# dusk-network/dusk-zerocaf

Measured on AMD Instinct MI355X. Metric: 252-bit Edwards variable-base scalar-muls/sec (batched, strict bit-exact mode), higher is better.
Workload: dtype u64 (nine 29-bit limbs in u32 registers, 64-bit multiply-accumulate columns); 1 GPU; 2^20 EdwardsPoint variable-base scalar-mul, random 252-bit scalars (BASELINE configs[2]); mode=strict (reference formula sequence, identical X:Y:Z:T limbs)

## Files before the change

### dusk_zerocaf_amd/csrc/zc_curve.hip.h

```cpp
#pragma once
#include "zc_arith.hip.h"

namespace zc {

typedef ModP FP;

struct pt {
    fe X, Y, Z, T;
};

template <int N>
struct exp_program {
    u32 e[N];
};
template <int N>
constexpr exp_program<N> make_program(const u32 (&src)[N])
{
    exp_program<N> p{};
    for (int i = 0; i < N; i++) p.e[i] = src[i];
    return p;
}
__device__ __constant__ exp_program<ModP::PROG_INV_LEN> ZC_PROG_INV = make_program(ModP::PROG_INV);
__device__ __constant__ exp_program<ModP::PROG_P58_LEN> ZC_PROG_P58 = make_program(ModP::PROG_P58);

// ... 587 lines not shown
    r.Ym = fp_sub(p.Y, p.X);
    r.Yp = fe_add(p.Y, p.X);
    r.Z = p.Z;
    r.T = p.T;
    return r;
}
ZC_DI ptm ptm_select(bool c, const ptm& a, const ptm& b)
{
    ptm r;
    r.Ym = fe_select(c, a.Ym, b.Ym);
    r.Yp = fe_select(c, a.Yp, b.Yp);
    r.Z = fe_select(c, a.Z, b.Z);
    r.T = fe_select(c, a.T, b.T);
    return r;
}
template <bool ILP = false>
ZC_DI ptm ptm_add(const ptm& p, const ptm& q)
{
    auto fp_mul = [](const fe& x, const fe& y) { return ILP ? mont_mul_ilp<FP>(x, y) : mont_mul<FP>(x, y); };
    const fe M = fp_mul(p.Ym, q.Ym);
    const fe P = fp_mul(p.Yp, q.Yp);
    const fe C = fp_mul(fp_mul_d(p.T), q.T);
    const fe D = fp_mul(p.Z, q.Z);
    const fe E = fe_sub_half<FP>(P, M);
    const fe H = fe_sub_lazy<FP>(P, E);
    const fe F = fe_sub_lazy<FP>(D, C);
    const fe G = fe_add(D, C);
    const fe X3 = fp_mul(E, F), Y3 = fp_mul(G, H);
    ptm r;
    r.Ym = fp_sub(Y3, X3);
    r.Yp = fe_add(Y3, X3);
    r.Z = fp_mul(F, G);
    r.T = fp_mul(E, H);
    return r;
}
ZC_DI pt ptm_to_pt(const ptm& p)
{
    const fe half = fe_const<FP>(ModP::INV2_M);
    pt r;
    r.X = fp_mul(fp_sub(p.Yp, fe_reduce<FP>(p.Ym)), half);
    r.Y = fp_mul(fe_add(p.Yp, p.Ym), half);
    r.Z = p.Z;
    r.T = p.T;
    return r;
}
ZC_DI pt pt_neg(const pt& p)
{
    pt r;
    r.X = fe_reduce<FP>(fp_neg(p.X));
    r.Y = p.Y;
    r.Z = p.Z;
    r.T = fe_reduce<FP>(fp_neg(p.T));
    return r;
}
ZC_DI pt pt_load(const u64* __restrict__ p)
{
    pt r;
    r.X = fe_load_mont<FP>(p);
    r.Y = fe_load_mont<FP>(p + 5);
    r.Z = fe_load_mont<FP>(p + 10);
    r.T = fe_load_mont<FP>(p + 15);
    return r;
}
ZC_DI void pt_store(u64* __restrict__ o, const pt& p)
{
    fe_store_canon<FP>(o, p.X);
    fe_store_canon<FP>(o + 5, p.Y);
    fe_store_canon<FP>(o + 10, p.Z);
    fe_store_canon<FP>(o + 15, p.T);
}

ZC_DI void scalar_effective(u64 (&l)[5])
{
#pragma unroll
    for (int j = 0; j < 5; j++) l[j] &= M52;
    const u64 low48 = ((u64)1 << 48) - 1;
    const u32 hi = (u32)(l[4] >> 48);
    if (hi) {
        const int tz = __builtin_ctz(hi);
        const bool stops_early = (l[1] | l[2] | l[3] | (l[4] & low48)) == 0 && l[0] < ((u64)1 << tz);
        if (stops_early) l[4] &= low48;
    }
}
ZC_DI void load_scalar(u64 (&l)[5], const u64* __restrict__ p)
{
    load5(l, p);
    scalar_effective(l);
}

ZC_DI void scalar_to_words(u32* __restrict__ sk, int stride, const u64 (&l)[5], int& nbits)
{
    u32 w[9];
#pragma unroll
    for (int k = 0; k < 9; k++) {
        const int bit = 32 * k, idx = bit / 52, sh = bit % 52;
        u64 x = (idx < 5) ? ((l[idx] & M52) >> sh) : 0;
        if (sh + 32 > 52 && idx + 1 < 5) x |= (l[idx + 1] & M52) << (52 - sh);
        w[k] = (u32)x;
    }
    w[8] &= 0xFu;
    nbits = 0;
#pragma unroll
    for (int k = 0; k < 9; k++) {
        if (w[k]) nbits = 32 * k + (32 - __builtin_clz(w[k]));
        sk[k * stride] = w[k];
    }
}

template <bool ILP = false>
ZC_DI pt scalar_mul_unified(const pt& P, const u32* __restrict__ sk, int stride, int nbits)
{
    ptm N = ptm_from_pt(P), Q = ptm_from_pt(pt_identity());
    int pos = 0;
    u32 cur = sk[0];
    bool pend = (cur & 1) != 0;
    bool active = nbits > 0;
    while (active) {
        const ptm lhs = ptm_select(pend, Q, N);
        const ptm r = ptm_add<ILP>(lhs, N);
        if (pend) {
            Q = r;
            pend = false;
            active = pos < nbits - 1;
        } else {
            N = r;
            pos++;
            if ((pos & 31) == 0) cur = sk[(pos >> 5) * stride];
            pend = ((cur >> (pos & 31)) & 1) != 0;
        }
    }
    return ptm_to_pt(Q);
}

ZC_DI ptm ptm_double_valid(const ptm& n)
{
    const fe M = mont_sqr<FP>(n.Ym);
    const fe P = mont_sqr<FP>(n.Yp);
    const fe D = mont_sqr<FP>(n.Z);
    const fe G = mont_mul<FP>(n.Ym, n.Yp);
    const fe E = fe_sub_half<FP>(P, M);
    const fe H = fe_sub_lazy<FP>(P, E);
    const fe F = fp_sub(fe_add(D, D), G);
    const fe X3 = mont_mul<FP>(E, F), Y3 = mont_mul<FP>(G, H);
    ptm r;
    r.Ym = fp_sub(Y3, X3);
    r.Yp = fe_add(Y3, X3);
    r.Z = mont_mul<FP>(F, G);
    r.T = mont_mul<FP>(E, H);
    return r;
}
ZC_DI bool pt_doubling_identities_hold(const pt& p, const ptm& n)
{
    const fe lhs = mont_mul<FP>(n.Ym, n.Yp);
    const fe rhs = fe_add(mont_sqr<FP>(p.Z), mont_mul<FP>(fe_const<FP>(ModP::D_M), mont_sqr<FP>(p.T)));
    return fp_eq(rhs, lhs) && fp_eq(mont_mul<FP>(p.T, p.Z), mont_mul<FP>(p.X, p.Y));
}
struct sm_lane {
    int pos, nbits;
    u32 cur;
    bool taken;
    bool has_stash;
    bool active;
};
ZC_DI sm_lane sm_lane_init(const u32* __restrict__ sk, int nbits)
{
    sm_lane L;
    L.pos = 0;
    L.nbits = nbits;
    L.cur = sk[0];
    L.taken = false;
    L.has_stash = false;
    L.active = nbits > 0;
    return L;
}
ZC_DI bool sm_bit_pending(const sm_lane& L) { return ((L.cur >> (L.pos & 31)) & 1) != 0 && !L.taken; }
ZC_DI bool sm_at_top(const sm_lane& L) { return L.active && L.pos >= L.nbits - 1; }
ZC_DI bool sm_tile_wants_d_step(bool any_active, bool any_at_top) { return any_active && !any_at_top; }
ZC_DI void sm_lane_advance(sm_lane& L, const u32* __restrict__ sk, int stride)
{
    L.pos++;
    if ((L.pos & 31) == 0) L.cur = sk[(L.pos >> 5) * stride];
    L.taken = false;
}
ZC_DI void sm_g_commit(ptm& dst, const u32 (&d)[9], const fe& Y3, const fe& X3, const fe& Z3, const fe& T3)
{
    u32 mask = M29, zero = 0;
    ZC_OPAQUE(mask);
    ZC_OPAQUE(zero);
#pragma unroll
    for (int i = 0; i < 9; i++) {
        dst.Ym.v[i] = i < 8 ? d[i] & mask : d[i];
        dst.Yp.v[i] = Y3.v[i] + X3.v[i] + zero;
    }
    dst.Z = Z3;
    dst.T = T3;
}
template <class STASH>
ZC_DI void sm_g_step(sm_lane& L, ptm& N, ptm& Q, const STASH& S, const u32* __restrict__ sk, int stride)
{
    const bool from_stash = L.active && L.has_stash;
    const bool add = L.active && (L.has_stash || sm_bit_pending(L));
    const bool dbl = L.active && !add;
    u32 d[9];
    fe X3, Y3, Z3, T3;
    {
        const ptm lhs = ptm_select(add, Q, N);
        const fe M = mont_mul<FP>(lhs.Ym, fe_select(from_stash, S.get(0), N.Ym));
        const fe P = mont_mul<FP>(lhs.Yp, fe_select(from_stash, S.get(1), N.Yp));
        const fe C = mont_mul<FP>(fp_mul_d(lhs.T), fe_select(from_stash, S.get(3), N.T));
        const fe D = mont_mul<FP>(lhs.Z, fe_select(from_stash, S.get(2), N.Z));
        const fe E = fe_sub_half<FP>(P, M);
        const fe H = fe_sub_lazy<FP>(P, E);
        const fe F = fe_sub_lazy<FP>(D, C);
        const fe G = fe_add(D, C);
        X3 = mont_mul<FP>(E, F);
        Y3 = mont_mul<FP>(G, H);
        Z3 = mont_mul<FP>(F, G);
        T3 = mont_mul<FP>(E, H);
    }
    for (int i = 0; i < 9; i++) ZC_ASSERT(X3.v[i] <= FP::BIAS[i] && Y3.v[i] < (1u << 31));
#pragma unroll
    for (int i = 0; i < 9; i++) d[i] = Y3.v[i] + (FP::BIAS[i] - X3.v[i]);
#pragma unroll
    for (int k = 0; k < 8; k++) d[k + 1] += d[k] >> 29;
    if (add) {
        sm_g_commit(Q, d, Y3, X3, Z3, T3);
        if (!from_stash) L.taken = true;
        L.has_stash = false;
    }
    if (dbl) {
        sm_g_commit(N, d, Y3, X3, Z3, T3);
        sm_lane_advance(L, sk, stride);
    }
    L.active = L.active && (L.pos < L.nbits - 1 || !L.taken);
}
template <class STASH>
ZC_DI void sm_d_step(sm_lane& L, ptm& N, STASH& S, const u32* __restrict__ sk, int stride)
{
    if (!L.active) return;
    if (sm_bit_pending(L)) {
        S.put(0, N.Ym);
        S.put(1, N.Yp);
        S.put(2, N.Z);
        S.put(3, N.T);
        L.has_stash = true;
    }
    N = ptm_double_valid(N);
    sm_lane_advance(L, sk, stride);
}

ZC_DI pt scalar_mul_ltr(const pt& P, const u32* __restrict__ pos_bits, const u32* __restrict__ neg_bits, int stride, int top)
{
    pt Q = pt_identity();
    pt Pn = P;
    Pn.X = fe_reduce<FP>(fp_neg(P.X));
    Pn.T = fe_reduce<FP>(fp_neg(P.T));
    int pos = top;
    bool active = top >= 0;
    bool pend = true;
    bool neg = active ? (((neg_bits[(top >> 5) * stride] >> (top & 31)) & 1) != 0) : false;
    while (active) {
        pt rhs = pt_select(neg, Pn, P);
        rhs = pt_select(pend, rhs, Q);
        Q = pt_add(Q, rhs);
        if (pend) {
            pend = false;
            active = pos > 0;
        } else {
            pos--;
            const u32 pw = pos_bits[(pos >> 5) * stride], nw = neg_bits[(pos >> 5) * stride];
            neg = ((nw >> (pos & 31)) & 1) != 0;
            pend = neg || (((pw >> (pos & 31)) & 1) != 0);
            active = pend || pos > 0;
        }
    }
    return Q;
}
template <int MODE>
ZC_DI int ltr_digits(u32* __restrict__ pos_bits, u32* __restrict__ neg_bits, int stride, const u64 (&l)[5])
{
    int top = -1;
    if (MODE == 1) {
        u32 w[9];
        int nb;
        scalar_to_words(w, 1, l, nb);
        w[7] &= 0x01FFFFFFu;
#pragma unroll
        for (int k = 0; k < 8; k++) {
            if (w[k]) top = 32 * k + (31 - __builtin_clz(w[k]));
            pos_bits[k * stride] = w[k];
            neg_bits[k * stride] = 0;
        }
        return top;
    }
    u64 k[5], m[5];
#pragma unroll
    for (int j = 0; j < 5; j++) k[j] = l[j] & M52;
    fe_to_limbs52(m, fe_const<ModL>(ModL::N));
    m[0] -= 1;
    u32 pcur = 0, ncur = 0;
    for (int i = 0; i < 256; i++) {
        const bool live = i < 250 && (k[0] | k[1] | k[2] | k[3] | k[4]) != 0;
        if (live && (k[0] & 1)) {
            if ((k[0] & 3) == 1) {
                k[0] -= 1;
                pcur |= 1u << (i & 31);
            } else {
// ... 681 lines not shown
```

### dusk_zerocaf_amd/csrc/zc_kernels.hip.h

```cpp
#pragma once
#include "zc_curve.hip.h"
#include "zc_msm_plan.h"
#include "zc_launch_plan.h"

namespace zc {

#define ZC_KERNEL extern "C" __global__ __launch_bounds__(256)
#define ZC_KERNEL_3W extern "C" __global__ __launch_bounds__(256) __attribute__((amdgpu_waves_per_eu(3)))
#define ZC_KERNEL_2W extern "C" __global__ __launch_bounds__(256) __attribute__((amdgpu_waves_per_eu(2)))

ZC_DI size_t gid() { return (size_t)blockIdx.x * ZC_BLOCK + threadIdx.x; }
ZC_DI int wave_max_i32(int v)
{
#pragma unroll
    for (int o = 32; o > 0; o >>= 1) {
        const int u = __shfl_xor(v, o);
        v = u > v ? u : v;
    }
    return v;
}

ZC_DI int wave_max_small(int v)
{
    int r = -1;
// ... 452 lines not shown
}
ZC_KERNEL void k_sc_invert_chunked(const u64* a, u64* out, uint8_t* ok, size_t n, int c)
{
    const size_t lanes = (n + (size_t)c - 1) / (size_t)c, g = gid();
    if (g < lanes) mod_invert_chunk<ModL, false>(a, out, ok, n, g, lanes, c);
}
ZC_KERNEL void k_sc_invert_chunked_lone(const u64* a, u64* out, uint8_t* ok, size_t n, int c)
{
    const size_t lanes = (n + (size_t)c - 1) / (size_t)c, g = gid();
    if (g < lanes) mod_invert_chunk<ModL, true>(a, out, ok, n, g, lanes, c);
}

ZC_KERNEL void k_ed_add(const u64* p, const u64* q, u64* out, size_t n)
{
    const size_t i = gid();
    if (i >= n) return;
    pt_store_plain(out + 20 * i, pt_add_plain(pt_load_plain(p + 20 * i), pt_load_plain(q + 20 * i)));
}
ZC_KERNEL void k_ed_sub(const u64* p, const u64* q, u64* out, size_t n)
{
    const size_t i = gid();
    if (i >= n) return;
    pt_store_plain(out + 20 * i, pt_add_plain(pt_load_plain(p + 20 * i), pt_neg(pt_load_plain(q + 20 * i))));
}
#ifndef ZC_ED_DOUBLE_SQR
#define ZC_ED_DOUBLE_SQR 1
#endif
ZC_KERNEL void k_ed_double(const u64* p, u64* out, size_t n)
{
    const size_t i = gid();
    if (i >= n) return;
    const pt a = pt_load_plain(p + 20 * i);
    pt_store_plain(out + 20 * i, ZC_ED_DOUBLE_SQR ? pt_double_plain(a) : pt_add_plain(a, a));
}
#ifndef ZC_ED_STAGED_EARLYQ
#define ZC_ED_STAGED_EARLYQ 1
#endif
#ifndef ZC_ED_STAGED_BLOCK
#define ZC_ED_STAGED_BLOCK 256
#endif
constexpr int ED_STAGED_BLOCK = ZC_ED_STAGED_BLOCK;
template <int OP>
ZC_DI void ed_binop_staged(const u64* p, const u64* q, u64* out, size_t n)
{
    constexpr int B = ED_STAGED_BLOCK;
    __shared__ __attribute__((aligned(16))) u64 sp[B * 20];
    const size_t base = (size_t)blockIdx.x * B;
    const int cnt = (int)((n - base < (size_t)B) ? (n - base) : (size_t)B);
    const int t = threadIdx.x;
    const u64x2* gp = reinterpret_cast<const u64x2*>(p + 20 * base);
    u64x2* lv = reinterpret_cast<u64x2*>(sp);
#if ZC_ED_STAGED_EARLYQ
    u64x2 qreg[10];
    if (OP != 2) {
        const u64x2* gq = reinterpret_cast<const u64x2*>(q + 20 * base);
#pragma unroll
        for (int k = 0; k < 10; k++) {
            const int v = t + k * B;
            if (v < cnt * 10) qreg[k] = gq[v];
        }
    }
#endif
    for (int v = t; v < cnt * 10; v += B) lv[v] = gp[v];
    __syncthreads();
    pt a = pt_identity(), b;
    if (t < cnt) a = pt_load_plain(sp + 20 * t);
    if (OP != 2) {
        __syncthreads();
#if ZC_ED_STAGED_EARLYQ
#pragma unroll
        for (int k = 0; k < 10; k++) {
            const int v = t + k * B;
            if (v < cnt * 10) lv[v] = qreg[k];
        }
#else
        const u64x2* gq = reinterpret_cast<const u64x2*>(q + 20 * base);
        for (int v = t; v < cnt * 10; v += B) lv[v] = gq[v];
#endif
        __syncthreads();
        b = pt_identity();
        if (t < cnt) b = pt_load_plain(sp + 20 * t);
        if (OP == 1) b = pt_neg(b);
    } else {
        b = a;
    }
    const pt r = OP == 2 && ZC_ED_DOUBLE_SQR ? pt_double_plain(a) : pt_add_plain(a, b);
    __syncthreads();
    if (t < cnt) pt_store_plain(sp + 20 * t, r);
    __syncthreads();
    u64x2* go = reinterpret_cast<u64x2*>(out + 20 * base);
    for (int v = t; v < cnt * 10; v += B) go[v] = lv[v];
}
#define ZC_KERNEL_EDS extern "C" __global__ __launch_bounds__(ZC_ED_STAGED_BLOCK)
ZC_KERNEL_EDS void k_ed_add_staged(const u64* p, const u64* q, u64* out, size_t n) { ed_binop_staged<0>(p, q, out, n); }
ZC_KERNEL_EDS void k_ed_sub_staged(const u64* p, const u64* q, u64* out, size_t n) { ed_binop_staged<1>(p, q, out, n); }
ZC_KERNEL_EDS void k_ed_double_staged(const u64* p, u64* out, size_t n) { ed_binop_staged<2>(p, nullptr, out, n); }
ZC_KERNEL_EDS void k_ed_neg_staged(const u64* p, u64* out, size_t n)
{
    constexpr int B = ED_STAGED_BLOCK;
    __shared__ __attribute__((aligned(16))) u64 sp[B * 20];
    const size_t base = (size_t)blockIdx.x * B;
    const int cnt = (int)((n - base < (size_t)B) ? (n - base) : (size_t)B);
    const int t = threadIdx.x;
    const u64x2* gp = reinterpret_cast<const u64x2*>(p + 20 * base);
    u64x2* lv = reinterpret_cast<u64x2*>(sp);
    for (int v = t; v < cnt * 10; v += B) lv[v] = gp[v];
    __syncthreads();
    if (t < cnt) {
        u64 m[5], X[5], T[5], nx[5], nt[5];
        const u64 z[5] = {0, 0, 0, 0, 0};
        limbs52_of_modulus<ModP>(m);
        load5(X, sp + 20 * t);
        load5(T, sp + 20 * t + 15);
        sub52(nx, z, X, m);
        sub52(nt, z, T, m);
        store5(sp + 20 * t, nx);
        store5(sp + 20 * t + 15, nt);
    }
    __syncthreads();
    u64x2* go = reinterpret_cast<u64x2*>(out + 20 * base);
    for (int v = t; v < cnt * 10; v += B) go[v] = lv[v];
}
ZC_KERNEL void k_ed_neg(const u64* p, u64* out, size_t n)
{
    const size_t i = gid();
    if (i >= n) return;
    u64 m[5], X[5], Y[5], Z[5], T[5], nx[5], nt[5];
    const u64 z[5] = {0, 0, 0, 0, 0};
    limbs52_of_modulus<ModP>(m);
    load5(X, p + 20 * i);
    load5(Y, p + 20 * i + 5);
    load5(Z, p + 20 * i + 10);
    load5(T, p + 20 * i + 15);
    sub52(nx, z, X, m);
    sub52(nt, z, T, m);
    store5(out + 20 * i, nx);
    store5(out + 20 * i + 5, Y);
    store5(out + 20 * i + 10, Z);
    store5(out + 20 * i + 15, nt);
}


ZC_DI u32 scalar_cost(const u64 (&l)[5])
{
    u32 bits = 0, pop = 0;
#pragma unroll
    for (int j = 0; j < 5; j++) {
        const u64 x = l[j] & M52;
        pop += __builtin_popcountll(x);
        if (x) bits = 52 * j + (64 - __builtin_clzll(x));
    }
    return bits ? bits - 1 + pop : 0;
}
ZC_KERNEL void k_sm_cost_hist(const u64* k, u32* hist, size_t n)
{
    __shared__ u32 h[ZC_COST_BINS];
    for (int b = threadIdx.x; b < ZC_COST_BINS; b += ZC_BLOCK) h[b] = 0;
    __syncthreads();
    const size_t i = gid();
    if (i < n) {
        u64 l[5];
        load_scalar(l, k + 5 * i);
        atomicAdd(&h[scalar_cost(l)], 1u);
    }
    __syncthreads();
    for (int b = threadIdx.x; b < ZC_COST_BINS; b += ZC_BLOCK)
        if (h[b]) atomicAdd(&hist[b], h[b]);
}
ZC_KERNEL void k_sm_cost_scan(u32* hist)
{
    __shared__ u32 part[ZC_BLOCK];
    const int t = threadIdx.x;
    u32 v[4], sum = 0;
#pragma unroll
    for (int j = 0; j < 4; j++) {
        v[j] = hist[ZC_COST_BINS - 1 - (4 * t + j)];
        sum += v[j];
    }
    part[t] = sum;
    __syncthreads();
    for (int d = 1; d < ZC_BLOCK; d <<= 1) {
        const u32 x = (t >= d) ? part[t - d] : 0;
        __syncthreads();
        part[t] += x;
        __syncthreads();
    }
    u32 base = part[t] - sum;
#pragma unroll
    for (int j = 0; j < 4; j++) {
        hist[ZC_COST_BINS - 1 - (4 * t + j)] = base;
        base += v[j];
    }
}
ZC_KERNEL void k_sm_cost_scatter(const u64* k, u32* offsets, u32* idx, size_t n)
{
    __shared__ u32 cnt[ZC_COST_BINS];
    __shared__ u32 base[ZC_COST_BINS];
    for (int b = threadIdx.x; b < ZC_COST_BINS; b += ZC_BLOCK) cnt[b] = 0;
    __syncthreads();
    const size_t i = gid();
    u32 c = 0, rank = 0;
    if (i < n) {
        u64 l[5];
        load_scalar(l, k + 5 * i);
        c = scalar_cost(l);
        rank = atomicAdd(&cnt[c], 1u);
    }
    __syncthreads();
    for (int b = threadIdx.x; b < ZC_COST_BINS; b += ZC_BLOCK)
        if (cnt[b]) base[b] = atomicAdd(&offsets[b], cnt[b]);
    __syncthreads();
    if (i < n) idx[base[c] + rank] = (u32)i;
}

ZC_DI int block_cost_rank(u32* __restrict__ skey, u32* __restrict__ sperm, u32 my_cost)
{
    const int tid = threadIdx.x;
    skey[tid] = my_cost;
    __syncthreads();
    int rank = 0;
    for (int u = 0; u < ZC_BLOCK; u++) {
        const u32 c = skey[u];
        rank += (c > my_cost || (c == my_cost && u < tid)) ? 1 : 0;
    }
    sperm[rank] = (u32)tid;
    __syncthreads();
    return (int)sperm[tid];
}

struct scalar_arg {
    u64 l[5];
};
ZC_KERNEL void k_ed_scalar_mul_bcast(const u64* p, scalar_arg k, u64* out, size_t n)
{
    __shared__ u32 sk[9 * ZC_BLOCK];
    const int tid = threadIdx.x;
    const size_t i = gid();
    const bool valid = i < n;
    int nbits;
    scalar_effective(k.l);
    scalar_to_words(sk + tid, ZC_BLOCK, k.l, nbits);
    const pt Q = scalar_mul_unified(pt_load(p + 20 * (valid ? i : 0)), sk + tid, ZC_BLOCK, valid ? nbits : 0);
    if (valid) pt_store(out + 20 * i, Q);
}

template <bool ILP>
ZC_DI void ed_scalar_mul_body(const u64* p, const u64* k, size_t k_stride, u64* out, size_t n)
{
    __shared__ u32 sk[9 * ZC_BLOCK];
    __shared__ u32 skey[ZC_BLOCK];
    __shared__ u32 sperm[ZC_BLOCK];
    __shared__ int snb[ZC_BLOCK];
    const int tid = threadIdx.x;
    const size_t i = gid();
    const bool valid = i < n;
    const size_t own = valid ? i : 0;
    u64 l[5];
    load_scalar(l, k + k_stride * own);
    int nbits;
    scalar_to_words(sk + tid, ZC_BLOCK, l, nbits);
    if (!valid) nbits = 0;
    int e = tid;
    if (k_stride != 0) {
        snb[tid] = nbits;
        e = block_cost_rank(skey, sperm, valid ? scalar_cost(l) : 0);
        nbits = snb[e];
    }
    const size_t base = (size_t)blockIdx.x * ZC_BLOCK;
    const bool run = base + e < n;
    const size_t ii = run ? base + e : 0;
    const pt P = pt_load(p + 20 * ii);
    const pt Q = scalar_mul_unified<ILP>(P, sk + e, ZC_BLOCK, run ? nbits : 0);
    if (run) pt_store(out + 20 * ii, Q);
}
ZC_KERNEL void k_ed_scalar_mul(const u64* p, const u64* k, size_t k_stride, u64* out, size_t n)
{
    ed_scalar_mul_body<false>(p, k, k_stride, out, n);
}
struct sm_stash_lds {
    u32* s;
    ZC_DI fe get(int c) const
    {
        fe r;
#pragma unroll
        for (int i = 0; i < 9; i++) r.v[i] = s[64 * (9 * c + i)];
        return r;
    }
    ZC_DI void put(int c, const fe& x) const
    {
#pragma unroll
        for (int i = 0; i < 9; i++) s[64 * (9 * c + i)] = x.v[i];
    }
};
ZC_KERNEL void k_ed_scalar_mul_pw(const u64* p, const u64* k, u64* out, const u32* idx, u32* counter, u32 n)
{
    __shared__ u32 sk[9 * ZC_BLOCK];
    __shared__ u32 st[36 * ZC_BLOCK];
    const int lane = threadIdx.x & 63;
    u32* skw = sk + 9 * (threadIdx.x & ~63) + lane;
    sm_stash_lds S;
    S.s = st + 36 * (threadIdx.x & ~63) + lane;
    const u32 ntiles = (n + 63) / 64;
    for (;;) {
        u32 t = 0;
        if (lane == 0) t = atomicAdd(counter, 1u);
        t = (u32)__builtin_amdgcn_readfirstlane((int)t);
        if (t >= ntiles) break;
        const u32 i = t * 64 + lane;
        const bool valid = i < n;
        const size_t own = valid ? (size_t)idx[i] : 0;
        u64 l[5];
        load_scalar(l, k + 5 * own);
        int nbits;
        scalar_to_words(skw, 64, l, nbits);
        const pt P = pt_load(p + 20 * own);
        ptm N = ptm_from_pt(P), Q = ptm_from_pt(pt_identity());
        const bool d_ok = wave_all(!valid || pt_doubling_identities_hold(P, N));
        sm_lane L = sm_lane_init(skw, valid ? nbits : 0);
        if (wave_any(L.active)) for (;;) {
            sm_g_step(L, N, Q, S, skw, 64);
            if (!wave_any(L.active)) break;
            if (d_ok && sm_tile_wants_d_step(true, wave_any(sm_at_top(L)))) sm_d_step(L, N, S, skw, 64);
        }
        if (valid) pt_store(out + 20 * own, ptm_to_pt(Q));
    }
}
ZC_KERNEL void k_ed_scalar_mul_pw_unified(const u64* p, const u64* k, u64* out, const u32* idx, u32* counter, u32 n)
{
    __shared__ u32 sk[9 * ZC_BLOCK];
    const int lane = threadIdx.x & 63;
    u32* skw = sk + 9 * (threadIdx.x & ~63) + lane;
    const u32 ntiles = (n + 63) / 64;
    for (;;) {
        u32 t = 0;
        if (lane == 0) t = atomicAdd(counter, 1u);
        t = (u32)__builtin_amdgcn_readfirstlane((int)t);
        if (t >= ntiles) break;
        const u32 i = t * 64 + lane;
        const bool valid = i < n;
        const size_t own = valid ? (size_t)idx[i] : 0;
        u64 l[5];
        load_scalar(l, k + 5 * own);
        int nbits;
        scalar_to_words(skw, 64, l, nbits);
        const pt Q = scalar_mul_unified<false>(pt_load(p + 20 * own), skw, 64, valid ? nbits : 0);
        if (valid) pt_store(out + 20 * own, Q);
    }
}
ZC_KERNEL void k_ed_scalar_mul_small(const u64* p, const u64* k, size_t k_stride, u64* out, size_t n)
{
    ed_scalar_mul_body<true>(p, k, k_stride, out, n);
}


ZC_DI u32 lane_id_fresh()
{
    u32 l;
    asm volatile("v_mbcnt_lo_u32_b32 %0, -1, 0\n\tv_mbcnt_hi_u32_b32 %0, -1, %0" : "=v"(l));
    return l;
}
struct ring_table {
    u32* base;
    ZC_DI u32* entry(int j) const
    {
        return base + (lane_id_fresh() * 256u + 32u * (u32)j);
// ... 631 lines not shown
```

### dusk_zerocaf_amd/csrc/zc_launch_plan.h

```cpp
#pragma once
#include <algorithm>
#include <cstddef>
#include <cstdint>

#include "zc_msm_plan.h"

namespace zc {

inline unsigned grid_for(size_t n) { return (unsigned)((n + ZC_BLOCK - 1) / ZC_BLOCK); }

enum LaunchForm {
    FORM_PER_LANE = 0,
    FORM_STAGED,
    FORM_STRICT_QUAD,
    FORM_STRICT_SMALL,
    FORM_STRICT_BLOCK,
    FORM_STRICT_PW,
    FORM_STRICT_PW_UNIFIED,
    FORM_INV_PER_ELEMENT,
    FORM_INV_CHUNKED,
    FORM_INV_LONE,
    LAUNCH_FORMS
};

constexpr size_t CHUNK_ROUND = (size_t)1 << 17;
constexpr size_t MAX_CHUNKS = 4096;
inline size_t host_chunk_elems(size_t cnt, bool heavy, long forced)
{
    size_t chunk = cnt;
    if (forced > 0)
        chunk = (cnt + forced - 1) / forced;
    else if (heavy && cnt >= 4 * CHUNK_ROUND)
        chunk = std::max(2 * CHUNK_ROUND, (cnt / 8 + CHUNK_ROUND - 1) / CHUNK_ROUND * CHUNK_ROUND);
    else if (heavy && cnt >= 2 * CHUNK_ROUND)
        chunk = CHUNK_ROUND;
    chunk = (chunk + 1023) / 1024 * 1024;
    return std::max(chunk, (cnt + MAX_CHUNKS - 1) / MAX_CHUNKS);
}

constexpr size_t STREAM_BYTES = (size_t)256 << 20;
constexpr size_t ED_STAGED_MIN_POINTS = (size_t)1 << 12;

struct StagedRule {
    size_t min_bytes = STREAM_BYTES;
    size_t min_rows = 0;
    unsigned block = ZC_BLOCK;
};
struct ElementwiseForm {
    LaunchForm form;
    unsigned block;
};
inline ElementwiseForm elementwise_form(size_t cnt, size_t limbs_per_row, size_t arrays, bool has_staged, const StagedRule& rule, long test_stream_min,
                                        bool all_aligned16)
{
    const size_t min_bytes = rule.min_bytes == STREAM_BYTES && test_stream_min > 0 ? (size_t)test_stream_min : rule.min_bytes;
    const bool staged = has_staged && cnt * sizeof(uint64_t) * limbs_per_row * arrays > min_bytes && cnt > rule.min_rows && all_aligned16;
    return staged ? ElementwiseForm{FORM_STAGED, rule.block} : ElementwiseForm{FORM_PER_LANE, (unsigned)ZC_BLOCK};
}

constexpr size_t BALANCE_MIN_N = 1 << 14;
constexpr int ZC_COST_BINS = 1024;
constexpr size_t BAL_COUNTERS = 64;
inline size_t balance_bytes(size_t cnt) { return (ZC_COST_BINS + BAL_COUNTERS + cnt) * sizeof(uint32_t); }
constexpr size_t PW_MIN_ELEMS = (size_t)1 << 17;
constexpr unsigned SMALL_LAUNCH_BLOCKS = 256;
constexpr size_t QUAD_LAUNCH_ELEMS = (size_t)1 << 14;

inline bool strict_wants_permutation(size_t cnt, bool sched_block)
{
    return cnt >= PW_MIN_ELEMS && !sched_block && cnt >= BALANCE_MIN_N && cnt <= 0xFFFFFFFFull;
}
struct StrictPlan {
    LaunchForm form;
    unsigned grid;
};
inline LaunchForm strict_kernel_for(size_t cnt) { return grid_for(cnt) <= SMALL_LAUNCH_BLOCKS ? FORM_STRICT_SMALL : FORM_STRICT_BLOCK; }
inline StrictPlan strict_form(size_t cnt, bool sched_unified, bool have_permutation, int cus, bool quad_ok = true)
{
    if (have_permutation) return {sched_unified ? FORM_STRICT_PW_UNIFIED : FORM_STRICT_PW, (unsigned)(3 * cus)};
    if (quad_ok && cnt <= QUAD_LAUNCH_ELEMS) return {FORM_STRICT_QUAD, (unsigned)((cnt + 63) / 64)};
    return {strict_kernel_for(cnt), grid_for(cnt)};
}

constexpr size_t INV_LANES_TARGET = 65536;
inline size_t inv_chunk(size_t cnt, long inv_chunk_knob)
{
    if (inv_chunk_knob) return (size_t)inv_chunk_knob;
    size_t c = cnt / INV_LANES_TARGET;
    return c > 32 ? 32 : c;
}
struct InversionPlan {
    LaunchForm form;
    size_t c;
    size_t lanes;
};
inline InversionPlan inversion_form(size_t cnt, bool in_place, long inv_chunk_knob, int cus)
{
    const size_t c = inv_chunk(cnt, inv_chunk_knob);
    if (c < 2 || in_place) return {FORM_INV_PER_ELEMENT, c, cnt};
    const size_t lanes = (cnt + c - 1) / c;
    return {lanes <= (size_t)cus * 256 ? FORM_INV_LONE : FORM_INV_CHUNKED, c, lanes};
}

constexpr uint32_t RING_XCDS = 8;
constexpr uint32_t RING_SLOTS = 512;
constexpr uint32_t RING_TICKET_STRIDE = 32;
constexpr uint32_t RING_STATE_WORDS = RING_XCDS * RING_TICKET_STRIDE + RING_XCDS * RING_SLOTS;
constexpr uint32_t RING_ERR_WORD = RING_STATE_WORDS;
constexpr uint32_t RING_ALLOC_WORDS = RING_STATE_WORDS + 32;
constexpr uint32_t RING_SLOT_DEAD = 0xFFFFFFFFu;
constexpr size_t RING_TABLE_BYTES = (size_t)RING_XCDS * RING_SLOTS * 64 * 1024;
constexpr size_t FAST_MAX_LAUNCH = (size_t)1 << 31;
constexpr size_t LINCOMB_MAX_UNITS = 2048;
inline size_t ring_units_per_xcd(size_t slot_units)
{
    return slot_units <= 1 ? (size_t)RING_SLOTS : std::min((size_t)RING_SLOTS * slot_units, LINCOMB_MAX_UNITS);
}
struct RingPlan {
    size_t units_per_xcd;
    uint32_t slots;
    size_t max_launch;
    size_t table_bytes;
};
inline RingPlan ring_plan(size_t slot_units, unsigned ring_slots_knob)
{
    const size_t units_per_xcd = ring_units_per_xcd(slot_units);
    const uint32_t slots = std::min(ring_slots_knob ? (uint32_t)ring_slots_knob : RING_SLOTS, (uint32_t)(units_per_xcd / slot_units));
    return {units_per_xcd, slots, std::min(FAST_MAX_LAUNCH, (size_t)slots << 24), RING_TABLE_BYTES / RING_SLOTS * units_per_xcd};
}
struct LincombLaunch {
    unsigned block;
    size_t lds_bytes;
};
inline LincombLaunch lincomb_launch(size_t slots_used)
{
    const unsigned block = slots_used > 4 ? 128u : (unsigned)ZC_BLOCK;
    return {block, 36 * slots_used * block};
}

inline bool hash_reader_words(size_t prefix_len, const size_t* part_len, const unsigned* ptr_mod8, size_t nparts, bool force_bytes)
{
    bool words = prefix_len % 8 == 0;
    for (size_t j = 0; j < nparts; j++) words = words && part_len[j] % 8 == 0 && ptr_mod8[j] == 0;
    return words && !force_bytes;
}

}
```

### dusk_zerocaf_amd/csrc/zerocaf_hip.hip

```cpp
#include <hip/hip_runtime.h>

#include <algorithm>
#include <atomic>
#include <cstdarg>
#include <cstdint>
#include <cstdio>
#include <cstdlib>
#include <cstring>
#include <initializer_list>
#include <map>
#include <memory>
#include <mutex>
#include <string>
#include <thread>
#include <type_traits>
#include <utility>
#include <vector>

#include <dlfcn.h>
#include <unistd.h>
#include <rccl/rccl.h>

#include "../../include/zerocaf_hip.h"
#include "../../include/zerocaf_hip_ext.h"
// ... 363 lines not shown
        long calls = 0;
        auto body = [&]() -> int {
            if (int rc0 = ring_check(ds)) return rc0;
            HIP_TRY(hipSetDevice(ds.device));
            void* base[MAX_ARGS] = {};
            for (int a = 0; a < nargs; a++) {
                if (!args[a].ptr) continue;
                if (int rc = ds.scratch[a].grow(args[a].elt_bytes * total)) return rc;
                base[a] = ds.scratch[a].as<void>();
            }
            while (ds.ev.size() < 2 * nchunks) {
                Event e;
                HIP_TRY(hipEventCreateWithFlags(e.put(), hipEventDisableTiming));
                ds.ev.push_back(std::move(e));
            }
            auto upload_and_launch = [&](size_t j) -> int {
                if (j >= nchunks) return ZC_OK;
                const size_t off = j * chunk, cnt = std::min(chunk, total - off);
                void* dptr[MAX_ARGS];
                for (int a = 0; a < nargs; a++) {
                    dptr[a] = base[a] ? (char*)base[a] + args[a].elt_bytes * off : nullptr;
                    if (!args[a].ptr || args[a].is_out) continue;
                    const char* src = (const char*)args[a].ptr + args[a].elt_bytes * (lo + off);
                    HIP_TRY(hipMemcpyAsync(dptr[a], src, args[a].elt_bytes * cnt, hipMemcpyHostToDevice, ds.copy_in));
                }
                HIP_TRY(hipEventRecord(ds.ev[2 * j], ds.copy_in));
                HIP_TRY(hipStreamWaitEvent(ds.s(), ds.ev[2 * j], 0));
                if (int lrc = launch_counted(dptr, cnt, ds, calls)) return lrc;
                HIP_TRY(hipGetLastError());
                HIP_TRY(hipEventRecord(ds.ev[2 * j + 1], ds.s()));
                return ZC_OK;
            };
            auto download = [&](size_t j) -> int {
                const size_t off = j * chunk, cnt = std::min(chunk, total - off);
                HIP_TRY(hipStreamWaitEvent(ds.copy_out, ds.ev[2 * j + 1], 0));
                for (int a = 0; a < nargs; a++) {
                    if (!args[a].ptr || !args[a].is_out) continue;
                    char* dst = (char*)const_cast<void*>(args[a].ptr) + args[a].elt_bytes * (lo + off);
                    HIP_TRY(hipMemcpyAsync(dst, (char*)base[a] + args[a].elt_bytes * off, args[a].elt_bytes * cnt, hipMemcpyDeviceToHost, ds.copy_out));
                }
                return ZC_OK;
            };
            constexpr size_t LOOKAHEAD = 2;
            int rc = ZC_OK;
            for (size_t j = 0; j < std::min(LOOKAHEAD, nchunks) && !rc; j++) rc = upload_and_launch(j);
            for (size_t j = 0; j < nchunks && !rc; j++) {
                rc = download(j);
                if (!rc) rc = upload_and_launch(j + LOOKAHEAD);
            }
            HIP_TRY(hipStreamSynchronize(ds.copy_in));
            HIP_TRY(hipStreamSynchronize(ds.s()));
            HIP_TRY(hipStreamSynchronize(ds.copy_out));
            if (!rc) rc = ring_check(ds);
            return rc;
        };
        const int rc = body();
        if (rc && err) *err = g_last_error;
        return rc;
    };

    if (ndev == 1 || n <= per) {
        std::string err;
        return device_job(0, &err);
    }
    std::vector<int> rcs(ndev, ZC_OK);
    std::vector<std::string> errs(ndev);
    std::vector<std::thread> workers;
    for (size_t di = 1; di < ndev; di++) workers.emplace_back([&, di] { rcs[di] = device_job(di, &errs[di]); });
    rcs[0] = device_job(0, &errs[0]);
    for (auto& t : workers) t.join();
    (void)hipSetDevice(ctx->devs[0].device);
    for (size_t di = 0; di < ndev; di++)
        if (rcs[di]) {
            g_last_error = errs[di];
            return rcs[di];
        }
    return ZC_OK;
}

#define REQUIRE(p) \
    if (!(p)) return fail(ZC_ERR_BAD_ARG, "null pointer: " #p)

template <class T>
struct Rows {
    T* ptr;
    size_t per;
    const char* name;
    bool optional;
};
template <class T>
inline Rows<T> rows(T* p, size_t per, const char* name, bool optional) { return Rows<T>{p, per, name, optional}; }
#define ROWS(p, per) rows(p, per, #p, false)
#define OPT_ROWS(p, per) rows(p, per, #p, true)

template <class Launch, size_t... I, class... T>
int batched_at(std::index_sequence<I...>, zc_ctx* ctx, size_t n, bool heavy, Launch& launch, const Rows<T>&... r)
{
    for (const char* missing : {(r.ptr || r.optional ? nullptr : r.name)...})
        if (missing) return failf(ZC_ERR_BAD_ARG, "null pointer: %s", missing);
    const Arg args[] = {Arg{r.ptr, sizeof(T) * r.per, !std::is_const<T>::value}...};
    return run_batched(ctx, args, (int)sizeof...(T), n, [&](void** d, size_t cnt, DevState& D) -> int { return launch(D, cnt, static_cast<T*>(d[I])...); }, heavy);
}
template <class Launch, class... T>
int batched(zc_ctx* ctx, size_t n, bool heavy, Launch&& launch, Rows<T>... r)
{
    static_assert(sizeof...(T) <= MAX_ARGS, "more buffers than a device slot has staging areas (MAX_ARGS)");
    return batched_at(std::index_sequence_for<T...>{}, ctx, n, heavy, launch, r...);
}
template <class... A>
auto plain(void (*k)(A...))
{
    return [k](DevState& D, size_t cnt, auto... p) -> int {
        static_assert(std::is_same<void (*)(A...), void (*)(decltype(p)..., size_t)>::value, "the buffers are not the kernel's parameters");
        hipLaunchKernelGGL(k, dim3(grid_for(cnt)), dim3(zc::ZC_BLOCK), 0, D.s(), p..., cnt);
        return ZC_OK;
    };
}

typedef void (*kbin_t)(const u64*, const u64*, u64*, size_t);
typedef void (*kun_t)(const u64*, u64*, size_t);

inline bool aligned16(const void* p) { return (reinterpret_cast<uintptr_t>(p) & 15) == 0; }

template <class K>
struct Staged {
    K kernel = nullptr;
    zc::StagedRule rule;
};
template <class K>
Staged<K> staged_points(K k) { return {k, {0, zc::ED_STAGED_MIN_POINTS, zc::ED_STAGED_BLOCK}}; }
template <class K, class... P>
int launch_elementwise(DevState& D, size_t cnt, size_t per, K k, const Staged<K>& st, P... p)
{
    const zc::ElementwiseForm f = zc::elementwise_form(cnt, per, sizeof...(p), st.kernel != nullptr, st.rule, D.tune.test_stream_min, (aligned16(p) && ...));
    count_form(D, f.form);
    hipLaunchKernelGGL(f.form == zc::FORM_STAGED ? st.kernel : k, dim3((unsigned)((cnt + f.block - 1) / f.block)), dim3(f.block), 0, D.s(), p..., cnt);
    return ZC_OK;
}
int binop(zc_ctx* ctx, kbin_t k, const uint64_t* a, const uint64_t* b, uint64_t* out, size_t n, size_t per, Staged<kbin_t> st = {})
{
    return batched(ctx, n, false, [&](DevState& D, size_t cnt, const u64* da, const u64* db, u64* dout) { return launch_elementwise(D, cnt, per, k, st, da, db, dout); },
                   ROWS(a, per), ROWS(b, per), ROWS(out, per));
}
int unop(zc_ctx* ctx, kun_t k, const uint64_t* a, uint64_t* out, size_t n, size_t per, Staged<kun_t> st = {})
{
    return batched(ctx, n, false, [&](DevState& D, size_t cnt, const u64* da, u64* dout) { return launch_elementwise(D, cnt, per, k, st, da, dout); },
                   ROWS(a, per), ROWS(out, per));
}

const zc::u32* balance_index(DevState& D, const u64* k, size_t cnt, zc::u32** counter)
{
    if (D.bal.grow(zc::balance_bytes(cnt)) != ZC_OK) return nullptr;
    zc::u32* hist = D.bal.as<zc::u32>();
    zc::u32* idx = hist + zc::ZC_COST_BINS + zc::BAL_COUNTERS;
    if (hipMemsetAsync(hist, 0, (zc::ZC_COST_BINS + zc::BAL_COUNTERS) * sizeof(zc::u32), D.s()) != hipSuccess) return nullptr;
    hipLaunchKernelGGL(zc::k_sm_cost_hist, dim3(grid_for(cnt)), dim3(zc::ZC_BLOCK), 0, D.s(), k, hist, cnt);
    hipLaunchKernelGGL(zc::k_sm_cost_scan, dim3(1), dim3(zc::ZC_BLOCK), 0, D.s(), hist);
    hipLaunchKernelGGL(zc::k_sm_cost_scatter, dim3(grid_for(cnt)), dim3(zc::ZC_BLOCK), 0, D.s(), k, hist, idx, cnt);
    *counter = hist + zc::ZC_COST_BINS;
    return idx;
}
template <class L>
int fast_ring(DevState& D, size_t cnt, L&& launch, size_t slot_units = 1)
{
    const zc::RingPlan ring = zc::ring_plan(slot_units, D.tune.ring_slots);
    if (int rc = D.fast.grow(ring.table_bytes)) return rc;
    if (!D.ring) {
        if (!D.ring_err) {
            hipError_t e = hipHostMalloc(D.ring_err.put(), 64, hipHostMallocMapped | hipHostMallocCoherent | hipHostMallocPortable);
            if (e != hipSuccess) return fail(ZC_ERR_NOMEM, "hipHostMalloc(ring error word)", e);
            *D.ring_error() = 0;
        }
        if (int rc = D.ring.alloc(zc::RING_ALLOC_WORDS * sizeof(zc::u32), "hipMalloc(ring state)")) return rc;
        void* dev_view = nullptr;
        hipError_t e = hipHostGetDevicePointer(&dev_view, (void*)D.ring_err, 0);
        const u64 addr = (u64)(uintptr_t)dev_view;
        if (e == hipSuccess) e = hipMemcpy(D.ring.as<zc::u32>() + zc::RING_ERR_WORD, &addr, sizeof addr, hipMemcpyHostToDevice);
        if (e != hipSuccess) {
            (void)D.ring.reset();
            return fail(ZC_ERR_HIP, "windowed core: ring state setup", e);
        }
    }
    zc::u32 slots_arg = ring.slots;
#ifdef ZC_TEST_HOOKS
    slots_arg |= (zc::u32)D.tune.test_ring_spins << 16;
#endif
    for (size_t off = 0; off < cnt; off += ring.max_launch) {
        HIP_TRY(hipMemsetAsync(D.ring.as<void>(), 0, zc::RING_STATE_WORDS * sizeof(zc::u32), D.s()));
        launch(D.fast.as<zc::u32>(), D.ring.as<zc::u32>(), slots_arg, off, std::min(ring.max_launch, cnt - off));
    }
#ifdef ZC_TEST_HOOKS
    if (D.tune.test_ring_poison) *D.ring_error() = 1;
#endif
    return ZC_OK;
}
int ring_check(DevState& D)
{
    volatile zc::u32* const err = D.ring_error();
    if (!err || *err == 0) return ZC_OK;
    *err = 0;
    return fail(ZC_ERR_HIP, "windowed core: a wave timed out waiting for its table slot; the rows it owned hold poison (all ones) -- "
                            "the outputs of the last windowed-core calls on this device are not valid");
}
void scalar_mul_on_device(DevState& D, const u64* p, const u64* k, u64* out, size_t cnt, bool quad_ok = true)
{
    zc::u32* counter = nullptr;
    const zc::u32* perm = zc::strict_wants_permutation(cnt, D.tune.sched_block) ? balance_index(D, k, cnt, &counter) : nullptr;
    const zc::StrictPlan sp = zc::strict_form(cnt, D.tune.sched_unified, perm != nullptr, D.cus, quad_ok);
    count_form(D, sp.form);
    switch (sp.form) {
    case zc::FORM_STRICT_PW:
    case zc::FORM_STRICT_PW_UNIFIED:
        hipLaunchKernelGGL(sp.form == zc::FORM_STRICT_PW_UNIFIED ? zc::k_ed_scalar_mul_pw_unified : zc::k_ed_scalar_mul_pw, dim3(sp.grid), dim3(zc::ZC_BLOCK), 0, D.s(), p, k, out,
                           perm, counter, (zc::u32)cnt);
        return;
    case zc::FORM_STRICT_QUAD:
        hipLaunchKernelGGL(zc::k_ed_scalar_mul_quad, dim3(sp.grid), dim3(zc::ZC_BLOCK), 0, D.s(), p, k, out, cnt);
        return;
    default:
        hipLaunchKernelGGL(sp.form == zc::FORM_STRICT_SMALL ? zc::k_ed_scalar_mul_small : zc::k_ed_scalar_mul, dim3(sp.grid), dim3(zc::ZC_BLOCK), 0, D.s(), p, k, (size_t)5, out, cnt);
    }
}
int scalar_mul_impl(zc_ctx* ctx, const uint64_t* p, const uint64_t* k, uint64_t* out, size_t n)
{
    return batched(ctx, n, true, [&](DevState& D, size_t cnt, const u64* dp, const u64* dk, u64* dout) {
        scalar_mul_on_device(D, dp, dk, dout, cnt);
        return ZC_OK;
    }, ROWS(p, 20), ROWS(k, 5), ROWS(out, 20));
}
int scalar_mul_bcast(zc_ctx* ctx, const uint64_t* p, const uint64_t (&k)[5], uint64_t* out, size_t n)
{
    zc::scalar_arg ka;
    for (int j = 0; j < 5; j++) ka.l[j] = k[j];
    return batched(ctx, n, true, [&](DevState& D, size_t cnt, const u64* dp, u64* dout) {
        hipLaunchKernelGGL(zc::k_ed_scalar_mul_bcast, dim3(grid_for(cnt)), dim3(zc::ZC_BLOCK), 0, D.s(), dp, ka, dout, cnt);
        return ZC_OK;
    }, ROWS(p, 20), ROWS(out, 20));
}

const u64* fold_all(DevState& D, u64* a, u64* b, size_t cnt)
{
    u64* cur = a;
    u64* nxt = b;
    while (cnt > 1) {
        hipLaunchKernelGGL(zc::k_ed_fold_pairs, dim3(grid_for((cnt + 1) / 2)), dim3(zc::ZC_BLOCK), 0, D.s(), (const u64*)cur, nxt, cnt);
        cnt = (cnt + 1) / 2;
        std::swap(cur, nxt);
    }
    return cur;
}

struct MsmWorkspace {
    zc::u32* digits;
    uint2* pairs_a;
    void* pairs_b;
    zc::u32 *sort_table, *sort_sums;
    zc::u32 *cached, *buckets;
    uint8_t* present;
    zc::u32 *ekeys[2], *erecs[2];
    u64 *seg_out, *fold_b, *out;
};
int msm_workspace(DevState& D, const MsmBucketPlan& p, size_t cached_points, size_t out_points, MsmWorkspace* ws, bool sort_only = false)
{
    const zc::MsmLayout l = zc::msm_workspace_layout(p, cached_points, out_points, sort_only);
    if (int rc = D.msm.grow(l.total)) return rc;
    char* const b = D.msm.as<char>();
    *ws = MsmWorkspace{(zc::u32*)(b + l.digits), (uint2*)(b + l.pairs_a), p.sort.passes == 1 ? nullptr : (void*)(b + l.pairs_b),
                       (zc::u32*)(b + l.sort_table), (zc::u32*)(b + l.sort_sums), (zc::u32*)(b + l.cached), (zc::u32*)(b + l.buckets),
                       (uint8_t*)(b + l.present), {(zc::u32*)(b + l.ekeys[0]), (zc::u32*)(b + l.ekeys[1])},
                       {(zc::u32*)(b + l.erecs[0]), (zc::u32*)(b + l.erecs[1])}, (u64*)(b + l.seg_out), (u64*)(b + l.fold_b), (u64*)(b + l.out)};
    return ZC_OK;
}

int msm_sort(DevState& D, hipStream_t st, const MsmSortPlan& pl, int w0, int nw, const zc::u32* digits, uint2* buf_a, void* buf_b, zc::u32* tables, size_t table_words,
             zc::u32* sums)
{
    const size_t base = (size_t)w0 * pl.pass[0].n;
    const zc::u32* in = digits + base;
    uint2* a = buf_a + base;
    void* b = !buf_b ? nullptr : pl.packed ? (void*)((zc::u32*)buf_b + base) : (void*)((uint2*)buf_b + base);
    void* out = (pl.passes & 1) ? (void*)a : b;
    for (int i = 0; i < pl.passes; i++) {
        zc::msm_sort_pass p = pl.pass[i];
        p.W = (zc::u32)nw;
        p.w0 = (zc::u32)w0;
        zc::u32* table = tables + (size_t)(i & 1) * table_words;
        const size_t words = zc::msm_sort_table_rows(p, (size_t)nw), padded = zc::msm_sort_table_words(p, (size_t)nw);
        const unsigned nblk = (unsigned)(padded / zc::SCAN_BLOCK_ELEMS), grid = (unsigned)(p.W * p.ncols);
        if (padded > words) HIP_TRY(hipMemsetAsync(table + words, 0, (padded - words) * sizeof(zc::u32), st));
        hipLaunchKernelGGL(!i ? zc::k_msm_sort_hist : pl.packed ? zc::k_msm_sort_hist_packed : zc::k_msm_sort_hist_pairs, dim3(grid), dim3(zc::ZC_BLOCK), 0, st, in, table, p);
        hipLaunchKernelGGL(zc::k_scan_reduce, dim3(nblk), dim3(zc::ZC_BLOCK), 0, st, (const zc::u32*)table, sums);
        hipLaunchKernelGGL(zc::k_scan_sums, dim3(1), dim3(zc::ZC_BLOCK), 0, st, sums, (zc::u32)nblk);
        hipLaunchKernelGGL(zc::k_scan_apply, dim3(nblk), dim3(zc::ZC_BLOCK), 0, st, table, (const zc::u32*)sums);
        if (pl.packed && i == 0)
            hipLaunchKernelGGL(zc::k_msm_sort_scatter_pack, dim3(grid), dim3(zc::ZC_BLOCK), 0, st, in, (zc::u32*)out, (const zc::u32*)table, p);
        else if (pl.packed)
            hipLaunchKernelGGL(zc::k_msm_sort_scatter_unpack, dim3(grid), dim3(zc::ZC_BLOCK), 0, st, in, (uint2*)out, (const zc::u32*)table,
                               (const zc::u32*)(tables + (size_t)((i - 1) & 1) * table_words), p);
        else
            hipLaunchKernelGGL(pl.big ? (i ? zc::k_msm_sort_scatter_pairs_big : zc::k_msm_sort_scatter_big) : (i ? zc::k_msm_sort_scatter_pairs : zc::k_msm_sort_scatter),
                               dim3(grid), dim3(zc::ZC_BLOCK), 0, st, in, (uint2*)out, (const zc::u32*)table, p);
        in = reinterpret_cast<const zc::u32*>(out);
        out = out == (void*)a ? b : (void*)a;
    }
    return ZC_OK;
}

int msm_fixed_check(size_t n, int window_bits, int* c_out, int* W_out, const char* who)
{
    if (n == 0) return failf(ZC_ERR_BAD_ARG, "%s: no bases", who);
    if (window_bits != 0 && (window_bits < zc::MSM_MIN_C || window_bits > zc::MSM_MAX_C))
        return failf(ZC_ERR_BAD_ARG, "%s: window_bits %d outside 0 or %d..%d", who, window_bits, zc::MSM_MIN_C, zc::MSM_MAX_C);
// ... 1605 lines not shown
```

Before: 61.66 million scalar-muls/s.

## Fuse cost histogram and scan via last-block ticket, persistent-grid prepass

Merges the cost-histogram and single-block scan kernels into one launch: each block bumps a global ticket after flushing its histogram, and the last block to finish runs the exclusive scan. The hist and scatter kernels now run a grid-stride loop over a grid capped at one block per CU, which cuts global atomic traffic. Scatter re-walks the scalars to place indices using per-block shared-memory cursors. It also replaces a generic constant multiply by d with fp_mul_d in a check helper. The aim is to remove one launch and shrink the balancing prepass overhead. The cost is a second pass over the scalars in scatter, and the order of indices within each bin is no longer deterministic.

```diff
diff --git a/dusk_zerocaf_amd/csrc/zc_curve.hip.h b/dusk_zerocaf_amd/csrc/zc_curve.hip.h
--- a/dusk_zerocaf_amd/csrc/zc_curve.hip.h
+++ b/dusk_zerocaf_amd/csrc/zc_curve.hip.h
@@ -763,7 +763,7 @@
 ZC_DI bool pt_doubling_identities_hold(const pt& p, const ptm& n)
 {
     const fe lhs = mont_mul<FP>(n.Ym, n.Yp);
-    const fe rhs = fe_add(mont_sqr<FP>(p.Z), mont_mul<FP>(fe_const<FP>(ModP::D_M), mont_sqr<FP>(p.T)));
+    const fe rhs = fe_add(mont_sqr<FP>(p.Z), fp_mul_d(mont_sqr<FP>(p.T)));
     return fp_eq(rhs, lhs) && fp_eq(mont_mul<FP>(p.T, p.Z), mont_mul<FP>(p.X, p.Y));
 }
 struct sm_lane {
diff --git a/dusk_zerocaf_amd/csrc/zc_kernels.hip.h b/dusk_zerocaf_amd/csrc/zc_kernels.hip.h
--- a/dusk_zerocaf_amd/csrc/zc_kernels.hip.h
+++ b/dusk_zerocaf_amd/csrc/zc_kernels.hip.h
@@ -628,29 +628,45 @@
     }
     return bits ? bits - 1 + pop : 0;
 }
-ZC_KERNEL void k_sm_cost_hist(const u64* k, u32* hist, size_t n)
+template <class F>
+ZC_DI void sm_cost_walk(const u64* k, size_t n, F f)
+{
+    const size_t stride = (size_t)gridDim.x * ZC_BLOCK;
+    for (size_t i = gid(); i < n; i += 4 * stride) {
+        u64 l[4][5];
+#pragma unroll
+        for (int u = 0; u < 4; u++)
+            if (i + u * stride < n) load_scalar(l[u], k + 5 * (i + u * stride));
+#pragma unroll
+        for (int u = 0; u < 4; u++)
+            if (i + u * stride < n) f(scalar_cost(l[u]), i + u * stride);
+    }
+}
+ZC_KERNEL void k_sm_cost_hist(const u64* k, u32* hist, u32* ticket, size_t n)
 {
     __shared__ u32 h[ZC_COST_BINS];
-    for (int b = threadIdx.x; b < ZC_COST_BINS; b += ZC_BLOCK) h[b] = 0;
+    __shared__ u32 part[ZC_BLOCK];
+    __shared__ u32 drawn;
+    const int t = threadIdx.x;
+    for (int b = t; b < ZC_COST_BINS; b += ZC_BLOCK) h[b] = 0;
     __syncthreads();
-    const size_t i = gid();
-    if (i < n) {
-        u64 l[5];
-        load_scalar(l, k + 5 * i);
-        atomicAdd(&h[scalar_cost(l)], 1u);
-    }
+    sm_cost_walk(k, n, [&](u32 c, size_t) { atomicAdd(&h[c], 1u); });
     __syncthreads();
-    for (int b = threadIdx.x; b < ZC_COST_BINS; b += ZC_BLOCK)
+    for (int b = t; b < ZC_COST_BINS; b += ZC_BLOCK)
         if (h[b]) atomicAdd(&hist[b], h[b]);
-}
-ZC_KERNEL void k_sm_cost_scan(u32* hist)
-{
-    __shared__ u32 part[ZC_BLOCK];
-    const int t = threadIdx.x;
+    asm volatile("s_waitcnt vmcnt(0)" ::: "memory");
+    __syncthreads();
+    if (t == 0) {
+        __threadfence();
+        asm volatile("s_waitcnt vmcnt(0)" ::: "memory");
+        drawn = __hip_atomic_fetch_add(ticket, 1u, __ATOMIC_RELAXED, __HIP_MEMORY_SCOPE_AGENT);
+    }
+    __syncthreads();
+    if (drawn != gridDim.x - 1) return;
     u32 v[4], sum = 0;
 #pragma unroll
     for (int j = 0; j < 4; j++) {
-        v[j] = hist[ZC_COST_BINS - 1 - (4 * t + j)];
+        v[j] = __hip_atomic_load(&hist[ZC_COST_BINS - 1 - (4 * t + j)], __ATOMIC_RELAXED, __HIP_MEMORY_SCOPE_AGENT);
         sum += v[j];
     }
     part[t] = sum;
@@ -670,23 +686,15 @@
 }
 ZC_KERNEL void k_sm_cost_scatter(const u64* k, u32* offsets, u32* idx, size_t n)
 {
-    __shared__ u32 cnt[ZC_COST_BINS];
-    __shared__ u32 base[ZC_COST_BINS];
-    for (int b = threadIdx.x; b < ZC_COST_BINS; b += ZC_BLOCK) cnt[b] = 0;
+    __shared__ u32 pos[ZC_COST_BINS];
+    for (int b = threadIdx.x; b < ZC_COST_BINS; b += ZC_BLOCK) pos[b] = 0;
     __syncthreads();
-    const size_t i = gid();
-    u32 c = 0, rank = 0;
-    if (i < n) {
-        u64 l[5];
-        load_scalar(l, k + 5 * i);
-        c = scalar_cost(l);
-        rank = atomicAdd(&cnt[c], 1u);
-    }
+    sm_cost_walk(k, n, [&](u32 c, size_t) { atomicAdd(&pos[c], 1u); });
     __syncthreads();
     for (int b = threadIdx.x; b < ZC_COST_BINS; b += ZC_BLOCK)
-        if (cnt[b]) base[b] = atomicAdd(&offsets[b], cnt[b]);
+        if (pos[b]) pos[b] = atomicAdd(&offsets[b], pos[b]);
     __syncthreads();
-    if (i < n) idx[base[c] + rank] = (u32)i;
+    sm_cost_walk(k, n, [&](u32 c, size_t i) { idx[atomicAdd(&pos[c], 1u)] = (u32)i; });
 }
 
 ZC_DI int block_cost_rank(u32* __restrict__ skey, u32* __restrict__ sperm, u32 my_cost)
diff --git a/dusk_zerocaf_amd/csrc/zc_launch_plan.h b/dusk_zerocaf_amd/csrc/zc_launch_plan.h
--- a/dusk_zerocaf_amd/csrc/zc_launch_plan.h
+++ b/dusk_zerocaf_amd/csrc/zc_launch_plan.h
@@ -62,6 +62,13 @@
 constexpr int ZC_COST_BINS = 1024;
 constexpr size_t BAL_COUNTERS = 64;
 inline size_t balance_bytes(size_t cnt) { return (ZC_COST_BINS + BAL_COUNTERS + cnt) * sizeof(uint32_t); }
+constexpr size_t BAL_TILE_COUNTER = 0;
+constexpr size_t BAL_PREPASS_TICKET = 32;
+constexpr unsigned PREPASS_BLOCKS_PER_CU = 1;
+inline unsigned prepass_grid(size_t cnt, int cus)
+{
+    return (unsigned)std::min<size_t>(grid_for(cnt), (size_t)PREPASS_BLOCKS_PER_CU * (size_t)std::max(cus, 1));
+}
 constexpr size_t PW_MIN_ELEMS = (size_t)1 << 17;
 constexpr unsigned SMALL_LAUNCH_BLOCKS = 256;
 constexpr size_t QUAD_LAUNCH_ELEMS = (size_t)1 << 14;
diff --git a/dusk_zerocaf_amd/csrc/zerocaf_hip.hip b/dusk_zerocaf_amd/csrc/zerocaf_hip.hip
--- a/dusk_zerocaf_amd/csrc/zerocaf_hip.hip
+++ b/dusk_zerocaf_amd/csrc/zerocaf_hip.hip
@@ -539,12 +539,14 @@
 {
     if (D.bal.grow(zc::balance_bytes(cnt)) != ZC_OK) return nullptr;
     zc::u32* hist = D.bal.as<zc::u32>();
-    zc::u32* idx = hist + zc::ZC_COST_BINS + zc::BAL_COUNTERS;
+    zc::u32* counters = hist + zc::ZC_COST_BINS;
+    zc::u32* idx = counters + zc::BAL_COUNTERS;
+    static_assert(zc::BAL_TILE_COUNTER < zc::BAL_COUNTERS && zc::BAL_PREPASS_TICKET < zc::BAL_COUNTERS, "the memset below covers BAL_COUNTERS words");
     if (hipMemsetAsync(hist, 0, (zc::ZC_COST_BINS + zc::BAL_COUNTERS) * sizeof(zc::u32), D.s()) != hipSuccess) return nullptr;
-    hipLaunchKernelGGL(zc::k_sm_cost_hist, dim3(grid_for(cnt)), dim3(zc::ZC_BLOCK), 0, D.s(), k, hist, cnt);
-    hipLaunchKernelGGL(zc::k_sm_cost_scan, dim3(1), dim3(zc::ZC_BLOCK), 0, D.s(), hist);
-    hipLaunchKernelGGL(zc::k_sm_cost_scatter, dim3(grid_for(cnt)), dim3(zc::ZC_BLOCK), 0, D.s(), k, hist, idx, cnt);
-    *counter = hist + zc::ZC_COST_BINS;
+    const unsigned grid = zc::prepass_grid(cnt, D.cus);
+    hipLaunchKernelGGL(zc::k_sm_cost_hist, dim3(grid), dim3(zc::ZC_BLOCK), 0, D.s(), k, hist, counters + zc::BAL_PREPASS_TICKET, cnt);
+    hipLaunchKernelGGL(zc::k_sm_cost_scatter, dim3(grid), dim3(zc::ZC_BLOCK), 0, D.s(), k, hist, idx, cnt);
+    *counter = counters + zc::BAL_TILE_COUNTER;
     return idx;
 }
 template <class L>
```

Measured after the change: 61.90 million scalar-muls/s, median of 6. Within noise of the previous version (+0.4%).
